# GreenleafLab/NucleoATAC

Measured on AMD Instinct MI355X. Metric: Mbp/s through occ+nuc signal pipeline, higher is better.
Workload: dtype f64

## Files before the change

### nucleoatac_amd/csrc/natac_api.hip

```cpp
#include "../../include/natac.h"
#ifndef NATAC_GNBL
#define NATAC_GNBL 2
#endif
#include "natac_kernels.hpp"
#include "natac_fft_bg.hpp"
#include "natac_occ_fast.hpp"
#include "natac_cand.hpp"
#include "natac_covsweep.hpp"
#include "natac_textz.hpp"
#include "natac_cores.hpp"
#include "natac_writer.hpp"
#include "natac_tabix.hpp"
#include "natac_pack.hpp"
#include "natac_bam.hpp"
#include "natac_bam_dev.hpp"
#include "natac_fragfile.hpp"
#include "natac_fragfile_dev.hpp"
#include "natac_fasta.hpp"
#include "natac_fuzzfit.hpp"
#include "natac_bedtab.hpp"
#include "natac_runtime.hpp"
#include "natac_pwmfit.hpp"
#include "natac_sites.hpp"
#include "natac_cellcounts.hpp"
// ... 6 lines not shown
#include "natac_peaks.hpp"
#include "natac_tracks.hpp"
#include "natac_dropins.hpp"
#include "natac_trackio.hpp"
#include "natac_files.hpp"
#include "natac_store.hpp"
#include "natac_profile.hpp"

#include <algorithm>
#include <cmath>
#include <cstdio>
#include <cstring>
#include <limits>
#include <string>
#include <vector>

using namespace natac;

static int need_nuc_geometry(const natac_batch *b, const char *who) {
    const natac_ctx *c = b->ctx;
    const BatchOutputs &o = b->out;
    if (o.nuc_w < 0 || (o.nuc_w == c->vw && o.nuc_lower == c->vlower && o.nuc_upper == c->vupper)) return NATAC_OK;
    return fail(NATAC_E_STATE, "%s: natac_run_nuc ran with the V-plot geometry lower=%d upper=%d w=%d, the context now holds lower=%d "
                "upper=%d w=%d: run natac_run_nuc again", who, o.nuc_lower, o.nuc_upper, o.nuc_w, c->vlower, c->vupper, c->vw);
}
static int need_occ_geometry(const natac_batch *b, const char *who) {
    const natac_ctx *c = b->ctx;
    const BatchOutputs &o = b->out;
    if (o.occ_step < 0 || (o.occ_step == c->step && o.occ_half == c->halfstep && o.occ_flank == c->flank && o.occ_upper == c->occ_upper))
        return NATAC_OK;
    return fail(NATAC_E_STATE, "%s: natac_run_occ ran with step=%d flank=%d upper=%d, the context now holds step=%d flank=%d upper=%d: "
                "run natac_run_occ again", who, o.occ_step, o.occ_flank, o.occ_upper, c->step, c->flank, c->occ_upper);
}

static int choose_bg_G(const natac_batch *b, int W) {
    const int cand[4] = {7, 9, 13, 17};
    double best = 1e300;
    int bestG = 9;
    const int stride = std::max(1, b->nc / 65536);
    for (int ci = 0; ci < 4; ++ci) {
        const int G = cand[ci], TW = 64 * G;
        double cost = 0;
        for (int i = 0; i < b->nc; i += stride) {
            const int nt = (b->h_len[i] + TW - 1) / TW;
            cost += (double)nt * (TW + (W - 1) * 0.15 * 8);
        }
        if (cost < best) { best = cost; bestG = G; }
    }
    return bestG;
}

static void launch_candidates(natac_ctx *c, const ChunkTable &ct, const VMatDev &vm, const int *d_cc, const int *d_cp, long long n,
                              const double *nuc_cov, const double *norm, const double *bnum, const double *bcov, double *lr,
                              double *var, double *z, const long long *tile_first = nullptr, const int2 *ranges256 = nullptr) {
    const int EW = c->W + ((c->vupper - 2) >> 1) + ((c->vupper - 1) >> 1);
    const int ZN = (((c->vupper - 2) >> 1) + ((c->vupper - 1) >> 1) + 5 + 32) & ~1, ON = (c->W + 1) & ~1;
    const size_t lds4 = ((size_t)4 * CAND_PER_WAVE * ((EW + 1) & ~1) + ZN + ON) * sizeof(double);
    const bool per_wave = c->W <= 2 * WAVE;
    const size_t ldsp = (size_t)4 * CAND_PER_WAVE * CANDP_STRIDE * sizeof(double);
    bool paired = per_wave && bnum && bcov && c->vlower >= 2 && (c->R & 1) == 0 && c->W >= 64 && !vm.has_zero && EW <= CANDP_STRIDE &&
                  !getenv("NATAC_CAND_FULL") && !getenv("NATAC_CAND_OLD");
    if (paired && (c->lrt_gen != c->model_gen || !c->d_lrt)) {
        if (c->d_lrt.size() < (size_t)c->R * c->W && dev_alloc(c->d_lrt, (size_t)c->R * c->W) != NATAC_OK)
            paired = false;
        if (paired) {
            hipLaunchKernelGGL(natac_lr_table, dim3((unsigned)((c->R * c->W + 255) / 256)), dim3(256), 0, c->stream, c->d_vmat, c->d_srow, c->R, c->W,
                               c->d_lrt);
            c->lrt_gen = c->model_gen;
        }
    }
    if (paired && (c->ctab_gen != c->model_gen || !c->d_ctab)) {
        const size_t nd = cand_table_doubles(c->R);
        if (c->d_ctab.size() < nd && dev_alloc(c->d_ctab, nd) != NATAC_OK) paired = false;
        if (paired) {
            hipLaunchKernelGGL(natac_cand_table, dim3((unsigned)((nd / 2 + 255) / 256)), dim3(256), 0, c->stream, c->d_vmat, c->R, c->W, c->d_ctab);
            c->ctab_gen = c->model_gen;
        }
    }
    if (paired) {
        VMatDev vml = vm;
        vml.lrt = c->d_lrt;
        vml.ctab = c->d_ctab;
        const long long per_block = 4 * CAND_PER_WAVE;
        const dim3 grid((unsigned)((n + per_block - 1) / per_block));
        if (c->vlower & 1)
            hipLaunchKernelGGL((natac_candidates_paired<true>), grid, dim3(256), ldsp, c->stream, ct, vml, d_cc, d_cp, (int)n, nuc_cov, norm,
                               bnum, bcov, tile_first, ranges256, lr, var, z);
        else
            hipLaunchKernelGGL((natac_candidates_paired<false>), grid, dim3(256), ldsp, c->stream, ct, vml, d_cc, d_cp, (int)n, nuc_cov, norm,
                               bnum, bcov, tile_first, ranges256, lr, var, z);
        return;
    }
    if (per_wave && lds4 <= 64 * 1024) {
        const long long per_block = 4 * CAND_PER_WAVE;
        if (bnum && bcov && !getenv("NATAC_CAND_FULL"))
            hipLaunchKernelGGL((natac_candidates4<true>), dim3((unsigned)((n + per_block - 1) / per_block)), dim3(256), lds4, c->stream,
                               ct, vm, d_cc, d_cp, (int)n, nuc_cov, norm, bnum, bcov, lr, var, z);
        else
            hipLaunchKernelGGL((natac_candidates4<false>), dim3((unsigned)((n + per_block - 1) / per_block)), dim3(256), lds4, c->stream,
                               ct, vm, d_cc, d_cp, (int)n, nuc_cov, norm, bnum, bcov, lr, var, z);
    } else {
        hipLaunchKernelGGL(natac_candidates, dim3((unsigned)n), dim3(256), (size_t)(EW + 2) * sizeof(double), c->stream, ct, vm, d_cc,
                           d_cp, nuc_cov, norm, lr, var, z);
    }
}

template <int G>
static void launch_bg(natac_batch *b, const ChunkTable &ct, const VMatDev &vm) {
    natac_ctx *c = b->ctx;
    constexpr int W = 121;
    const int PW = 64 * G + W - 1;
    const int EW = PW + ((vm.upper - 2) >> 1) + ((vm.upper - 1) >> 1);
    const size_t lds = ((size_t)((EW + 1) & ~1) + PW) * sizeof(double);
    hipLaunchKernelGGL((natac_background<G, W>), dim3(b->n_tiles_bg), dim3(64), lds, c->stream, ct, b->d_tiles_bg, vm,
                       b->d_track[NATAC_T_NUC_COV], b->d_track[NATAC_T_RAW], b->d_track[NATAC_T_BACKGROUND],
                       b->d_track[NATAC_T_NORM], b->d_bnum, b->d_bcov);
}

struct OccFastLaunch { natac_batch *b; const ChunkTable &ct; const OccFastDev &of; size_t lds_gs, lds_od; int rem; bool rn16; };
template <int STEP, int REM = 0>
static void occ_gsum_launch(const OccFastLaunch &f) {
    if constexpr (REM < STEP) {
        if (f.rem == REM)
            hipLaunchKernelGGL((natac_occ_gsum<STEP, REM>), dim3(f.b->n_tiles_gs), dim3(256), f.lds_gs, f.b->ctx->stream, f.ct, f.b->d_tiles_gs, f.of,
                               f.b->d_blk_off, f.b->total_blocks, f.b->d_gsum);
        else
            occ_gsum_launch<STEP, REM + 1>(f);
    }
}
template <int STEP>
static void occ_fast_launch(const OccFastLaunch &f) {
    natac_batch *b = f.b;
    occ_gsum_launch<STEP>(f);
    auto kd = (f.of.flags & 2) ? (f.rn16 ? natac_occ_decide<STEP, 16, true> : natac_occ_decide<STEP, 4, true>)
                               : (f.rn16 ? natac_occ_decide<STEP, 16, false> : natac_occ_decide<STEP, 4, false>);
    const bool heavy_first = b->ctx->occ_ordered;
    hipLaunchKernelGGL(kd, dim3((b->n_tiles_occ + (heavy_first ? HEAVY_CAP : 0) + 3) / 4), dim3(256), f.lds_od, b->ctx->stream, f.ct, b->d_tiles_occ,
                       b->n_tiles_occ, b->d_ranges_occ, heavy_first ? b->d_order_occ : nullptr, f.of, b->d_blk_off, b->total_blocks, b->d_gsum, b->d_grid[0], b->d_grid[1], b->d_grid[2], b->d_defer,
                       b->d_defer + 1);
}

extern "C" {

// ... 395 lines not shown
    o.zero_flags = c->occ_zero_flags;
    o.b_floor = c->occ_b_floor;
    return o;
}

static int build_tiles(natac_batch *b, int width, PoolBuf<int2> &d_out, int *n_out, bool grid_units = false, int step = 1, int half = 0) {
    std::vector<int2> tiles;
    tiles.reserve((size_t)(b->total_bp / std::max(1, width)) + b->nc);
    for (int i = 0; i < b->nc; ++i) {
        int n = b->h_len[i];
        if (grid_units) n = (b->h_len[i] > half) ? (b->h_len[i] - half + step - 1) / step : 0;
        for (int x = 0; x < n; x += width) tiles.push_back(make_int2(i, x));
    }
    *n_out = (int)tiles.size();
    int rc = dev_upload(b->ctx, d_out, tiles.data(), tiles.size());
    if (rc) return rc;
    HIPCHK(sync_all(b->ctx));
    return NATAC_OK;
}

int natac_batch_create(natac_ctx *c, int32_t nc, const int32_t *chunk_len, const int64_t *frag_off, const int32_t *frag_lpos,
                       const int32_t *frag_ilen, const int64_t *bias_off, const double *bias_log, int32_t bias_left,
                       int32_t bias_right, natac_batch **out) {
    if (!c || !out || !chunk_len || !frag_off) return fail(NATAC_E_ARG, "null argument");
    *out = nullptr;
    if (nc <= 0) return fail(NATAC_E_ARG, "n_chunks must be positive");
    if (bias_log && !bias_off) return fail(NATAC_E_ARG, "bias_log without bias_off");
    if (frag_off[0] != 0) return fail(NATAC_E_ARG, "frag_off[0] must be 0");
    const long long nf = frag_off[nc];
    if (nf > 0 && (!frag_lpos || !frag_ilen)) return fail(NATAC_E_ARG, "fragment arrays are NULL");
    HIPCHK(hipSetDevice(c->device));
    natac_batch *b = new natac_batch();
    b->ctx = c; b->nc = nc; b->nf = nf; b->bias_left = bias_left; b->bias_right = bias_right;
    b->h_len.assign(chunk_len, chunk_len + nc);
    b->h_out_off.resize((size_t)nc + 1);
    b->h_out_off[0] = 0;
    for (int i = 0; i < nc; ++i) {
        if (chunk_len[i] <= 0) { delete b; return fail(NATAC_E_ARG, "chunk %d has length %d", i, chunk_len[i]); }
        if (frag_off[i + 1] < frag_off[i] || frag_off[i + 1] - frag_off[i] > 0x7fffffffLL) {
            delete b; return fail(NATAC_E_ARG, "frag_off not monotone (chunk %d)", i);
        }
        if (bias_off && bias_off[i + 1] - bias_off[i] != (long long)chunk_len[i] + bias_left + bias_right) {
            delete b; return fail(NATAC_E_ARG, "bias slice of chunk %d must cover [start-%d, end+%d)", i, bias_left, bias_right);
        }
        b->h_out_off[i + 1] = b->h_out_off[i] + chunk_len[i];
        b->max_len = std::max(b->max_len, chunk_len[i]);
    }
    b->total_bp = b->h_out_off[nc];
    b->nb = bias_off ? bias_off[nc] : 0;
    auto upload = [&]() -> int {
        int rc;
        if ((rc = dev_upload(c, b->d_len, chunk_len, (size_t)nc)) ||
            (rc = dev_upload(c, b->d_frag_off, (const long long *)frag_off, (size_t)nc + 1)) ||
            (rc = dev_upload(c, b->d_lpos, frag_lpos, (size_t)nf)) || (rc = dev_upload(c, b->d_ilen, frag_ilen, (size_t)nf)) ||
            (rc = dev_alloc(b->d_centre, (size_t)nf)) || (rc = dev_upload(c, b->d_out_off, b->h_out_off.data(), (size_t)nc + 1)))
            return rc;
        if (bias_off) {
            if ((rc = dev_upload(c, b->d_bias_off, (const long long *)bias_off, (size_t)nc + 1))) return rc;
            if (bias_log) rc = dev_upload(c, b->d_bias, bias_log, (size_t)b->nb);
            else rc = dev_alloc(b->d_bias, (size_t)b->nb);
            if (rc) return rc;
        }
        if ((rc = dev_alloc(b->d_status, (size_t)nc))) return rc;
        hipError_t e = hipMemsetAsync(b->d_status, 0, (size_t)nc * sizeof(int), c->stream);
        if (e != hipSuccess) return fail(NATAC_E_HIP, "memset: %s", hipGetErrorString(e));
        if (nf > 0) {
            int blocks = (int)std::min<long long>((nf + 255) / 256, 4096);
            hipLaunchKernelGGL(natac_frag_centres, dim3(blocks), dim3(256), 0, c->stream, b->d_lpos, b->d_ilen, b->d_centre, nf);
        }
        if ((rc = build_tiles(b, 256, b->d_tiles256, &b->n_tiles256))) return rc;
        {
            std::vector<long long> first((size_t)nc + 1, 0);
            for (int i = 0; i < nc; ++i) first[(size_t)i + 1] = first[i] + (chunk_len[i] + 255) / 256;
            if ((rc = dev_upload(c, b->d_tile256_first, first.data(), first.size()))) return rc;
        }
        e = hipStreamSynchronize(c->stream);
        if (e != hipSuccess) return fail(NATAC_E_HIP, "upload: %s", hipGetErrorString(e));
        return NATAC_OK;
    };
    if (int rc = upload()) {
        natac_batch_free(b);
        return rc;
    }
    *out = b;
    return NATAC_OK;
}

int natac_batch_create_from_seq(natac_ctx *c, int32_t nc, const int32_t *chunk_len, const int64_t *frag_off, const int32_t *frag_lpos,
                                const int32_t *frag_ilen, const int64_t *seq_off, const uint8_t *seq, const double *log_pwm,
                                const uint8_t *nucleotides, int nrow, int K, int32_t bias_left, int32_t bias_right, natac_batch **out) {
    if (!c || !out || !chunk_len || !seq_off || !seq || !log_pwm || !nucleotides) return fail(NATAC_E_ARG, "null argument");
    if (nc <= 0 || nrow < 1 || K < 1) return fail(NATAC_E_ARG, "bad argument");
    std::vector<int64_t> boff((size_t)nc + 1, 0);
    for (int i = 0; i < nc; ++i) {
        const int64_t nb = (int64_t)chunk_len[i] + bias_left + bias_right;
        if (seq_off[i + 1] - seq_off[i] != nb + K - 1)
            return fail(NATAC_E_ARG, "sequence window of chunk %d must hold %lld bases ([start-%d-up, end+%d+down))", i, (long long)(nb + K - 1),
                        bias_left, bias_right);
        boff[(size_t)i + 1] = boff[(size_t)i] + nb;
    }
    int rc = natac_batch_create(c, nc, chunk_len, frag_off, frag_lpos, frag_ilen, boff.data(), nullptr, bias_left, bias_right, out);
    if (rc) return rc;
    natac_batch *b = *out;
    DeviceCall dc(c, "pwm score");
    const unsigned char *d_s = dc.upload((const unsigned char *)seq, (size_t)seq_off[nc]);
    const long long *d_so = dc.upload((const long long *)seq_off, (size_t)nc + 1);
    const unsigned char *d_n = dc.upload((const unsigned char *)nucleotides, (size_t)nrow);
    const double *d_p = dc.upload(log_pwm, (size_t)nrow * K);
    if (dc.ok()) {
// ... 577 lines not shown
    for (int r = 1; r < nrow; ++r)
        for (int q = 0; q < r; ++q)
            if (nucleotides[q] == nucleotides[r]) return fail(NATAC_E_ARG, "PWM rows %d and %d have the same letter", q, r);
    if (seq_off[0] != 0) return fail(NATAC_E_ARG, "seq_off[0] must be 0");
    for (int i = 0; i < b->nc; ++i)
        if (seq_off[i + 1] - seq_off[i] != (int64_t)b->h_len[i] + K - 1)
            return fail(NATAC_E_ARG, "sequence window of chunk %d must hold %lld bases (its length + K - 1)", i, (long long)b->h_len[i] + K - 1);
    natac_ctx *c = b->ctx;
    DeviceCall dc(c, "pwm_track");
    int rc;
    if (!dc.ok()) return dc.finish();
    if ((rc = ensure_track(b, NATAC_T_BIAS)) || (rc = ensure_tiles1k(b))) return rc;
    const unsigned char *d_s = dc.upload((const unsigned char *)seq, (size_t)seq_off[b->nc]);
    const long long *d_so = dc.upload((const long long *)seq_off, (size_t)b->nc + 1);
    const unsigned char *d_n = dc.upload((const unsigned char *)nucleotides, (size_t)nrow);
    const double *d_p = dc.upload(log_pwm, (size_t)nrow * K);
    if (dc.ok()) {
        dc.prof_begin(NATAC_K_PWM_TRACK);
        hipLaunchKernelGGL(natac_pwm_track, dim3(b->n_tiles1k), dim3(TR_BLOCK), pwm_track_lds(nrow, K), c->stream, b->d_tiles1k.get(), b->d_len.get(),
                           d_so, d_s, b->d_out_off.get(), d_p, d_n, nrow, K, b->d_track[NATAC_T_BIAS].get());
        dc.prof_end();
        dc.launched();
    }
    if ((rc = dc.finish())) return rc;
    b->out.track[NATAC_T_BIAS] = TS_RUN;
    return NATAC_OK;
}

static int need_candidate_inputs(natac_batch *b) {
    int rc;
    if ((rc = need_track(b, NATAC_T_NUC_COV)) || (rc = need_track(b, NATAC_T_NORM))) return rc;
    if (b->d_bias && !b->d_ebias) return fail(NATAC_E_STATE, "natac_run_nuc must run before the candidate statistics (exp(bias))");
    return NATAC_OK;
}

int natac_run_candidates(natac_batch *b, int64_t n_cand, const int32_t *cand_chunk, const int32_t *cand_pos, double *lr,
                         double *var, double *z) {
    if (!b) return fail(NATAC_E_ARG, "batch is NULL");
    natac_ctx *c = b->ctx;
    int rc = need_candidate_inputs(b);
    if (rc || (rc = need_nuc_geometry(b, "natac_run_candidates"))) return rc;
    if (n_cand < 0 || (n_cand > 0 && (!cand_chunk || !cand_pos || !lr || !var || !z))) return fail(NATAC_E_ARG, "null argument");
    if (n_cand == 0) return NATAC_OK;
    if (n_cand > 0x7fffffffLL) return fail(NATAC_E_ARG, "too many candidates");
    DeviceCall dc(c, "candidates");
    if (!dc.ok()) return dc.finish();
    for (int64_t k = 0; k < n_cand; ++k) {
        const int ci = cand_chunk[k];
        if (ci < 0 || ci >= b->nc || cand_pos[k] < 0 || cand_pos[k] >= b->h_len[ci])
            return fail(NATAC_E_ARG, "candidate %lld out of range (chunk %d pos %d)", (long long)k, ci, cand_pos[k]);
    }
    if ((rc = ensure_srow(c))) return rc;
    const int *d_cc = dc.upload(cand_chunk, (size_t)n_cand), *d_cp = dc.upload(cand_pos, (size_t)n_cand);
    double *d_out = dc.alloc<double>((size_t)3 * n_cand);
    if (dc.ok()) {
        const ChunkTable ct = make_table(b);
        const VMatDev vm = make_vmat(c);
        dc.prof_begin(NATAC_K_CAND);
        launch_candidates(c, ct, vm, d_cc, d_cp, n_cand, b->d_track[NATAC_T_NUC_COV], b->d_track[NATAC_T_NORM],
                          b->out.bg_gen == c->model_gen ? b->d_bnum : nullptr, b->out.bg_gen == c->model_gen ? b->d_bcov : nullptr, d_out,
                          d_out + n_cand,
                          d_out + 2 * n_cand, b->ranges256_w == c->vw ? b->d_tile256_first : nullptr, b->ranges256_w == c->vw ? b->d_ranges256 : nullptr);
        dc.prof_end();
        dc.launched();
    }
    dc.fetch(lr, d_out, (size_t)n_cand);
    dc.fetch(var, d_out + n_cand, (size_t)n_cand);
    dc.fetch(z, d_out + 2 * n_cand, (size_t)n_cand);
    return dc.finish();
}

int natac_run_candidates_cov(natac_batch *b, int64_t n_cand, const int32_t *cand_chunk, const int32_t *cand_pos, int mode,
                             double *var) {
    if (!b) return fail(NATAC_E_ARG, "batch is NULL");
    natac_ctx *c = b->ctx;
    int rc = need_track(b, NATAC_T_NUC_COV);
    if (rc || (rc = need_nuc_geometry(b, "natac_run_candidates_cov"))) return rc;
    if (mode < 0 || mode > 2) return fail(NATAC_E_ARG, "mode must be 0 (closed form), 1 (literal) or 2 (closed form in fp32)");
    if (n_cand < 0 || (n_cand > 0 && (!cand_chunk || !cand_pos || !var))) return fail(NATAC_E_ARG, "null argument");
    if (n_cand == 0) return NATAC_OK;
    DeviceCall dc(c, "candidates_cov");
    if (!dc.ok()) return dc.finish();
    for (int64_t k = 0; k < n_cand; ++k) {
        const int ci = cand_chunk[k];
        if (ci < 0 || ci >= b->nc || cand_pos[k] < 0 || cand_pos[k] >= b->h_len[ci])
            return fail(NATAC_E_ARG, "candidate %lld out of range (chunk %d pos %d)", (long long)k, ci, cand_pos[k]);
    }
    if ((rc = ensure_srow(c))) return rc;
    const int N = c->R * c->W;
    const int NBLK = 64;
    const int64_t SLAB = 2048;
    const ChunkTable ct = make_table(b);
    const VMatDev vm = make_vmat(c);
    const int EW = c->W + ((c->vupper - 2) >> 1) + ((c->vupper - 1) >> 1);
    const int64_t slab = std::min<int64_t>(SLAB, n_cand);
    std::vector<double> part((size_t)slab * NBLK);
    int *d_cc = dc.alloc<int>((size_t)slab), *d_cp = dc.alloc<int>((size_t)slab);
    double *d_p = dc.alloc<double>((size_t)slab * N), *d_out = dc.alloc<double>((size_t)slab * NBLK);
    for (int64_t k0 = 0; k0 < n_cand; k0 += slab) {
        const int64_t m = std::min<int64_t>(slab, n_cand - k0);
        const int per = mode == 1 ? NBLK : 1;
        dc.send(d_cc, cand_chunk + k0, (size_t)m);
        dc.send(d_cp, cand_pos + k0, (size_t)m);
        if (dc.ok()) {
            hipLaunchKernelGGL(natac_cand_window_probs, dim3((unsigned)m), dim3(256), (size_t)(EW + 2) * sizeof(double), c->stream, ct, vm,
                               d_cc, d_cp, d_p);
            dc.launched();
        }
        if (dc.ok()) {
            if (mode == 1)
                hipLaunchKernelGGL(natac_cov_literal_many, dim3(NBLK, (unsigned)m), dim3(256), 0, c->stream, d_p, c->d_vmat, N, d_out);
            else if (mode == 0)
                hipLaunchKernelGGL((natac_cov_closed_many<double>), dim3((unsigned)m), dim3(256), 0, c->stream, d_p, c->d_vmat, N, d_out);
            else
                hipLaunchKernelGGL((natac_cov_closed_many<float>), dim3((unsigned)m), dim3(256), 0, c->stream, d_p, c->d_vmat, N, d_out);
// ... 33 lines not shown
    natac_ctx *c = b->ctx;
    if (order < 1 || order > 255 || sep < 1 || boundary < 0) return fail(NATAC_E_ARG, "bad peak parameters");
    const int maxL = b->max_len;
    if (n_jitter < maxL) return fail(NATAC_E_ARG, "jitter stream (%lld) shorter than the longest chunk (%d)", (long long)n_jitter, maxL);
    HIPCHK(hipSetDevice(c->device));
    HIPCHK(sync_all(c));
    int rc;
    if (with_stats && (rc = ensure_srow(c))) return rc;
    if (!b->d_jitter || b->n_jitter < maxL) {
        if ((rc = dev_upload(c, b->d_jitter, jitter, (size_t)maxL))) return rc;
        HIPCHK(hipStreamSynchronize(c->stream));
        b->n_jitter = maxL;
    } else {
        HIPCHK(hipMemcpyAsync(b->d_jitter, jitter, (size_t)maxL * sizeof(double), hipMemcpyHostToDevice, c->stream));
        HIPCHK(hipStreamSynchronize(c->stream));
    }
    if (b->pk_order != order) {
        std::vector<long long> cap((size_t)b->nc + 1, 0);
        for (int i = 0; i < b->nc; ++i) cap[i + 1] = cap[i] + b->h_len[i] / (order + 1) + 2;
        b->slot_total = cap[b->nc];
        b->d_cap_off.reset(); b->d_slot.reset();
        if ((rc = dev_upload(c, b->d_cap_off, cap.data(), (size_t)b->nc + 1))) return rc;
        HIPCHK(hipStreamSynchronize(c->stream));
        if ((rc = dev_alloc(b->d_slot, (size_t)b->slot_total))) return rc;
        b->pk_order = order;
    }
    if (!b->d_pk_count && (rc = dev_alloc(b->d_pk_count, (size_t)b->nc))) return rc;
    if (!b->d_pk_offs && (rc = dev_alloc(b->d_pk_offs, (size_t)b->nc + 1))) return rc;
    if (form_smooth &&
        (rc = ensure_window(c, c->d_win_nuc, &c->win_nuc_M, &c->win_nuc_sd, b->out.smooth_M, b->out.smooth_sd, &c->win_nuc_sum))) return rc;
    const PeakPlan plan = peaks_plan(maxL, order);
    PeakSearch s{sig_a, sig_b, b->d_jitter, min_signal, boundary, order, sep, b->d_cap_off, b->d_slot, b->d_pk_count, b->d_status,
                 b->d_pk_offs, c->d_win_nuc, c->win_nuc_sum, form_smooth ? b->d_track[NATAC_T_SMOOTH].get() : nullptr};
    if (plan.global_lists) {
        if (b->d_pk_big.size() < (size_t)b->slot_total * 2 + 2 && (rc = dev_alloc(b->d_pk_big, (size_t)b->slot_total * 2 + 2))) return rc;
        s.big_sig = b->d_pk_big;
        s.big_pos = (int *)(b->d_pk_big + b->slot_total);
        s.big_state = (unsigned char *)(s.big_pos + b->slot_total);
    }
    natac_ctx::Ev ev;
    prof_begin(c, NATAC_K_CAND, ev);
    const ChunkTable ct = make_table(b);
    if ((rc = peaks_enqueue(plan, ct, b->nc, s, c->stream))) return rc;
    long long total = 0;
    HIPCHK(hipGetLastError());
    if (form_smooth) b->out.track[NATAC_T_SMOOTH] = TS_RUN;
    HIPCHK(hipMemcpyAsync(&total, b->d_pk_offs + b->nc, sizeof(long long), hipMemcpyDeviceToHost, c->stream));
    HIPCHK(hipStreamSynchronize(c->stream));
    if (total > b->pk_cap) {
        b->d_pk_chunk.reset(); b->d_pk_pos.reset(); b->d_pk_out.reset();
        b->pk_cap = 0;
        const long long cap = total + total / 4 + 16;
        if ((rc = dev_alloc(b->d_pk_chunk, (size_t)cap)) || (rc = dev_alloc(b->d_pk_pos, (size_t)cap)) ||
            (rc = dev_alloc(b->d_pk_out, (size_t)3 * cap))) {
            b->d_pk_chunk.reset(); b->d_pk_pos.reset();
            return rc;
        }
        b->pk_cap = cap;
    }
    if (total > 0) {
        hipLaunchKernelGGL(natac_compact_candidates, dim3((b->nc + 3) / 4), dim3(256), 0, c->stream, b->nc, b->d_pk_count, b->d_pk_offs,
                           b->d_cap_off, b->d_slot, b->d_pk_chunk, b->d_pk_pos);
        if (with_stats) {
            const VMatDev vm = make_vmat(c);
            launch_candidates(c, ct, vm, b->d_pk_chunk, b->d_pk_pos, total, b->d_track[NATAC_T_NUC_COV], b->d_track[NATAC_T_NORM],
                              b->out.bg_gen == c->model_gen ? b->d_bnum : nullptr, b->out.bg_gen == c->model_gen ? b->d_bcov : nullptr,
                              b->d_pk_out, b->d_pk_out + b->pk_cap, b->d_pk_out + 2 * b->pk_cap,
                              b->ranges256_w == c->vw ? b->d_tile256_first : nullptr, b->ranges256_w == c->vw ? b->d_ranges256 : nullptr);
        }
    }
    b->pk_has_stats = with_stats;
    prof_end(c, ev);
    HIPCHK(hipGetLastError());
    b->pk_n = total;
    *n_cand = total;
    return NATAC_OK;
}

int natac_peaks_plan(int32_t max_len, int32_t order, int32_t *kernel, int32_t *bt, int32_t *nj, int32_t *mask, int32_t *global_lists,
                     int32_t *forms_smooth, int32_t *pk_cap, int64_t *lds_bytes) {
    if (!kernel || !bt || !nj || !mask || !global_lists || !forms_smooth || !pk_cap || !lds_bytes) return fail(NATAC_E_ARG, "null argument");
    if (max_len < 1 || order < 1 || order > 255) return fail(NATAC_E_ARG, "natac_peaks_plan: a positive length and an order in 1..255");
    const PeakPlan p = peaks_plan(max_len, order);
    *kernel = p.kernel; *bt = p.bt; *nj = p.nj; *mask = p.mask; *global_lists = p.global_lists; *forms_smooth = p.forms_smooth;
    *pk_cap = p.pk_cap;
    lds_bytes[0] = (int64_t)p.lds; lds_bytes[1] = (int64_t)p.lds_smooth;
    return NATAC_OK;
}

int natac_run_peaks(natac_batch *b, double min_signal, int sep, int boundary, int order, const double *jitter, int64_t n_jitter,
                    int64_t *n_cand) {
    if (!b) return fail(NATAC_E_ARG, "batch is NULL");
    int rc;
    const bool form_smooth = b->out.track[NATAC_T_SMOOTH] == TS_PENDING && peaks_smooth_arm(b, order);
    if ((!form_smooth && (rc = need_track(b, NATAC_T_SMOOTH))) || (rc = need_candidate_inputs(b)) ||
        (rc = need_nuc_geometry(b, "natac_run_peaks"))) return rc;
    return run_peaks_impl(b, b->d_track[NATAC_T_NORM], b->d_track[NATAC_T_SMOOTH], true, min_signal, sep, boundary, order, jitter,
                          n_jitter, n_cand, form_smooth);
}

int natac_run_track_peaks(natac_batch *b, int track, double min_signal, int sep, int boundary, int order, const double *jitter,
                          int64_t n_jitter, int64_t *n_peaks) {
    if (!b) return fail(NATAC_E_ARG, "batch is NULL");
    if (track == NATAC_T_INS) return fail(NATAC_E_ARG, "peak search needs a float64 track");
    int rc = need_track(b, track);
    if (rc) return rc;
    return run_peaks_impl(b, b->d_track[track], nullptr, false, min_signal, sep, boundary, order, jitter, n_jitter, n_peaks);
}

int natac_run_occ_peaks(natac_batch *b, double min_occ, int sep, const double *jitter, int64_t n_jitter, int64_t *n_peaks) {
    if (!b || !n_peaks) return fail(NATAC_E_ARG, "null argument");
    int rc;
    for (int t : {NATAC_T_OCC, NATAC_T_OCC_LOWER, NATAC_T_OCC_UPPER, NATAC_T_OCC_COV}) if ((rc = need_track(b, t))) return rc;
    if ((rc = need_occ_geometry(b, "natac_run_occ_peaks"))) return rc;
    natac_ctx *c = b->ctx;
    const int U = c->occ_upper;
    if (U > 1024) return fail(NATAC_E_ARG, "upper > 1024");
    rc = run_peaks_impl(b, b->d_track[NATAC_T_OCC], nullptr, false, min_occ, sep, sep / 2, 1, jitter, n_jitter, n_peaks);
    if (rc) return rc;
    const long long n = *n_peaks;
// ... 177 lines not shown
```

### nucleoatac_amd/csrc/natac_cand.hpp

```cpp
#pragma once
#include "natac_kernels.hpp"

namespace natac {

__device__ __forceinline__ int row_lower_bound(const int *__restrict__ a, int lo, int hi, int key, int l, int sh) {
    while (__ballot(hi - lo > 16) != 0ull) {
        const int n = hi - lo;
        const bool big = n > 16;
        const int stride = big ? (n + 15) / 16 : 1;
        const int pi = min((l + 1) * stride - 1, max(n - 1, 0));
        const bool less = big && a[lo + pi] < key;
        const int cnt = __popc((unsigned)(__ballot(less) >> sh) & 0xffffu);
        if (big) {
            lo = min(lo + cnt * stride, hi);
            hi = min(lo + stride, hi);
        }
    }
    const int i = lo + l;
    const bool less = (i < hi) && a[i] < key;
    return lo + __popc((unsigned)(__ballot(less) >> sh) & 0xffffu);
}

__global__ void __launch_bounds__(256) natac_lr_table(const double *__restrict__ vmat, const double *__restrict__ srow, int R, int W,
                                                        double *__restrict__ out) {
    const int i = blockIdx.x * 256 + threadIdx.x;
    if (i < R * W) out[i] = log(vmat[i] / srow[i / W]);
}

constexpr int CAND_TAB_PAD = 2;
constexpr int CAND_TAB_PAIR = WAVE * 4;
__host__ __device__ constexpr size_t cand_table_doubles(int R) { return (size_t)((R >> 1) + CAND_TAB_PAD) * CAND_TAB_PAIR; }
__global__ void __launch_bounds__(256) natac_cand_table(const double *__restrict__ vmat, int R, int W, double *__restrict__ out) {
    const int i = blockIdx.x * 256 + threadIdx.x;
    const int k = i >> 7, row = (i >> 6) & 1, l = i & 63;
    if (k >= (R >> 1) + CAND_TAB_PAD) return;
    double v0 = 0.0, v1 = 0.0;
    if (k < (R >> 1)) {
        const double *r = vmat + (size_t)(2 * k + row) * W;
        v0 = r[l];
        if (l + WAVE < W) v1 = r[l + WAVE];
    }
    out[(size_t)i * 2] = v0;
    out[(size_t)i * 2 + 1] = v1;
}

constexpr int CANDP_STRIDE = 376;

template <bool LODD>
__global__ void __launch_bounds__(256) __attribute__((amdgpu_waves_per_eu(3, 3))) natac_candidates_paired(
    ChunkTable ct, VMatDev vm, const int *__restrict__ cand_chunk, const int *__restrict__ cand_pos, int ncand,
    const double *__restrict__ nuc_cov, const double *__restrict__ norm, const double *__restrict__ bnum,
    const double *__restrict__ bcov, const long long *__restrict__ tile_first, const int2 *__restrict__ ranges256,
    double *__restrict__ out_lr, double *__restrict__ out_var, double *__restrict__ out_z) {
    extern __shared__ __attribute__((aligned(16))) double smem[];
    constexpr int Q = CAND_PER_WAVE;
    const int A = (vm.upper - 2) >> 1, Bh = (vm.upper - 1) >> 1;
    const int W = vm.W, R = vm.R;
    const int EW = W + A + Bh;
    constexpr int EWP = CANDP_STRIDE;
    const int wave = threadIdx.x >> 6, lane = threadIdx.x & 63;
    double *Ew = smem + wave * Q * EWP;
    const int k0 = (blockIdx.x * 4 + wave) * Q;
    if (k0 >= ncand) return;
    constexpr int NT = (CANDP_STRIDE + WAVE - 1) / WAVE;
    int chunk[Q], pos[Q];
#pragma unroll
    for (int q = 0; q < Q; ++q) {
        const int k = (k0 + q < ncand) ? k0 + q : k0;
        chunk[q] = cand_chunk[k];
        pos[q] = cand_pos[k];
    }
    double ev[Q][NT];
    if (ct.bias) {
        int nb[Q];
        const double *b[Q];
#pragma unroll
        for (int q = 0; q < Q; ++q) {
            nb[q] = ct.chunk_len[chunk[q]] + ct.bias_left + ct.bias_right;
            b[q] = ct.ebias + ct.bias_off[chunk[q]];
        }
#pragma unroll
        for (int q = 0; q < Q; ++q) {
            const int j0 = pos[q] - vm.w - A + ct.bias_left + lane;
#pragma unroll
            for (int t = 0; t < NT; ++t) ev[q][t] = b[q][min(max(j0 + WAVE * t, 0), nb[q] - 1)];
        }
#pragma unroll
        for (int q = 0; q < Q; ++q) {
            const int j0 = pos[q] - vm.w - A + ct.bias_left + lane;
#pragma unroll
            for (int t = 0; t < NT; ++t) {
                const int j = j0 + WAVE * t;
                ev[q][t] = (j >= 0 && j < nb[q]) ? ev[q][t] : 0.0;
            }
        }
    } else {
#pragma unroll
        for (int q = 0; q < Q; ++q)
#pragma unroll
            for (int t = 0; t < NT; ++t) ev[q][t] = 1.0;
    }
    bool esmall = false;
#pragma unroll
    for (int q = 0; q < Q; ++q) {
        double emin = __builtin_inf();
#pragma unroll
        for (int t = 0; t < NT; ++t) {
            const int u = lane + WAVE * t;
            if (u < EW) {
                Ew[q * EWP + u] = ev[q][t];
                emin = fmin(emin, ev[q][t]);
            }
        }
        esmall |= !(wave_min(emin) > 0x1p-500);
    }
    __builtin_amdgcn_wave_barrier();
    const int c1 = lane, c2 = min(lane + WAVE, W - 1);
    const bool h2 = lane + WAVE < W;
    double a1[Q][2], a2[Q][2];
    double carry[Q][2];
#pragma unroll
    for (int q = 0; q < Q; ++q) { a1[q][0] = a1[q][1] = a2[q][0] = a2[q][1] = 0.0; }
    const int m0 = LODD ? (vm.lower - 1) >> 1 : vm.lower >> 1;
    {
        const int off = LODD ? A + m0 : A - m0 + 1;
#pragma unroll
        for (int q = 0; q < Q; ++q) { carry[q][0] = Ew[q * EWP + c1 + off]; carry[q][1] = Ew[q * EWP + c2 + off]; }
    }
    const double *__restrict__ vmat = vm.mat;
    const int npair = R >> 1;
    constexpr int DSH = LODD ? -1 : 1, DNW = LODD ? 1 : -1;
    constexpr int BSH = DSH < 0 ? 3 : 0, BNW = DNW < 0 ? 3 : 0;
    const int ew0 = wave * Q * EWP;
    int ish1 = ew0 + c1 + (LODD ? A - m0 : A + m0) - BSH, ish2 = ew0 + c2 + (LODD ? A - m0 : A + m0) - BSH;
    int inw1 = ew0 + c1 + (LODD ? A + m0 + 1 : A - m0) - BNW, inw2 = ew0 + c2 + (LODD ? A + m0 + 1 : A - m0) - BNW;
    asm("" : "+v"(ish1), "+v"(ish2), "+v"(inw1), "+v"(inw2));
    struct PairT { double va0, va1, vb0, vb1, sa, sb; };
    constexpr int PAIRB = CAND_TAB_PAIR * (int)sizeof(double);
    const char *ctab = (const char *)vm.ctab;
    unsigned vo = (unsigned)lane * 16u + 4u * PAIRB;
    asm("" : "+v"(vo));
    auto load_pair = [&](int kk, int imm) {
        const double2 *p = (const double2 *)(ctab + (size_t)vo + (ptrdiff_t)imm);
        const double2 a = p[0], b = p[WAVE];
        return PairT{a.x, a.y, b.x, b.y, vm.srow[2 * kk], vm.srow[2 * kk + 1]};
    };
    auto pair_step = [&](const PairT &t, const double (&cin)[Q][2], double (&cout)[Q][2], auto osh, auto onw) {
        const double va0 = t.va0, va1 = t.va1, vb0 = t.vb0, vb1 = t.vb1;
        const double wa0 = t.sa * (va0 * va0), wa1 = t.sa * (va1 * va1);
        const double wb0 = t.sb * (vb0 * vb0), wb1 = t.sb * (vb1 * vb1);
        double s0[Q], s1[Q];
#pragma unroll
        for (int q = 0; q < Q; ++q) {
            s0[q] = smem[ish1 + (q * EWP + osh)]; s1[q] = smem[ish2 + (q * EWP + osh)];
            cout[q][0] = smem[inw1 + (q * EWP + onw)]; cout[q][1] = smem[inw2 + (q * EWP + onw)];
        }
        __builtin_amdgcn_sched_barrier(0);
#pragma unroll
        for (int q = 0; q < Q; ++q) {
            const double n0 = cout[q][0], n1 = cout[q][1];
            a1[q][0] = fma(s0[q], fma(vb0, n0, va0 * cin[q][0]), a1[q][0]);
            a1[q][1] = fma(s1[q], fma(vb1, n1, va1 * cin[q][1]), a1[q][1]);
            a2[q][0] = fma(s0[q], fma(wb0, n0, wa0 * cin[q][0]), a2[q][0]);
            a2[q][1] = fma(s1[q], fma(wb1, n1, wa1 * cin[q][1]), a2[q][1]);
        }
    };
#define NATAC_OFF(J, B, D) std::integral_constant<int, (B) + (J) * (D)>{}
    double carry2[Q][2];
    int k = 0;
    PairT t0 = load_pair(0, -4 * PAIRB), t1 = load_pair(min(1, npair - 1), -3 * PAIRB);
    for (; k + 4 <= npair; k += 4) {
        const PairT u0 = load_pair(min(k + 2, npair - 1), -2 * PAIRB);
        pair_step(t0, carry, carry2, NATAC_OFF(0, BSH, DSH), NATAC_OFF(0, BNW, DNW));
        const PairT u1 = load_pair(min(k + 3, npair - 1), -PAIRB);
        pair_step(t1, carry2, carry, NATAC_OFF(1, BSH, DSH), NATAC_OFF(1, BNW, DNW));
        t0 = load_pair(min(k + 4, npair - 1), 0);
        pair_step(u0, carry, carry2, NATAC_OFF(2, BSH, DSH), NATAC_OFF(2, BNW, DNW));
        t1 = load_pair(min(k + 5, npair - 1), PAIRB);
        pair_step(u1, carry2, carry, NATAC_OFF(3, BSH, DSH), NATAC_OFF(3, BNW, DNW));
        ish1 += 4 * DSH; ish2 += 4 * DSH; inw1 += 4 * DNW; inw2 += 4 * DNW;
        vo += 4u * PAIRB;
    }
    ish1 += BSH; ish2 += BSH; inw1 += BNW; inw2 += BNW;
    for (; k + 2 <= npair; k += 2) {
        pair_step(t0, carry, carry2, NATAC_OFF(0, 0, DSH), NATAC_OFF(0, 0, DNW));
        t0 = load_pair(min(k + 2, npair - 1), -2 * PAIRB);
        pair_step(t1, carry2, carry, NATAC_OFF(1, 0, DSH), NATAC_OFF(1, 0, DNW));
        t1 = load_pair(min(k + 3, npair - 1), -PAIRB);
        ish1 += 2 * DSH; ish2 += 2 * DSH; inw1 += 2 * DNW; inw2 += 2 * DNW;
        vo += 2u * PAIRB;
    }
    if (k < npair) pair_step(t0, carry, carry2, NATAC_OFF(0, 0, DSH), NATAC_OFF(0, 0, DNW));
#undef NATAC_OFF
    bool zero[Q];
#pragma unroll
    for (int q = 0; q < Q; ++q) zero[q] = false;
    if (esmall) {
        for (int r = 0; r < R; ++r) {
            const int i = vm.lower + r;
            const int hl = floor_half(i - 1), hr = floor_half(i);
            const double sr = vm.srow[r];
            const double v1 = vmat[r * W + c1], v2 = vmat[r * W + c2];
#pragma unroll
            for (int q = 0; q < Q; ++q) {
                const double *e = Ew + q * EWP;
                const double b1 = e[c1 + A - hl] * e[c1 + A + hr], b2 = e[c2 + A - hl] * e[c2 + A + hr];
                zero[q] |= (v1 * b1 == 0.0 || sr * b1 == 0.0) || (h2 && (v2 * b2 == 0.0 || sr * b2 == 0.0));
            }
        }
    }
    double tBV2[Q], tB0V[Q];
    bool anyzero[Q];
#pragma unroll
    for (int q = 0; q < Q; ++q) {
        tB0V[q] = wave_sum(a1[q][0] + a1[q][1]);
        tBV2[q] = wave_sum(a2[q][0] + a2[q][1]);
        anyzero[q] = __ballot(zero[q]) != 0ull;
    }
    const int row = lane >> 4, l = lane & 15, sh = 16 * row;
    int mych = chunk[0], myp = pos[0];
    double myB0V = tB0V[0], myBV2 = tBV2[0];
    bool myzero = anyzero[0];
#pragma unroll
    for (int q = 1; q < Q; ++q)
        if (row == q) { mych = chunk[q]; myp = pos[q]; myB0V = tB0V[q]; myBV2 = tBV2[q]; myzero = anyzero[q]; }
    const long long op = ct.out_off[mych] + myp;
    const double tB = bcov[op], tBV = bnum[op];
    const int nfr = (int)(ct.frag_off[mych + 1] - ct.frag_off[mych]);
    const int *cen = ct.centre + ct.frag_off[mych];
    const int *iln = ct.ilen + ct.frag_off[mych];
    int f0, f1;
    if (ranges256) {
        const int2 tr = ranges256[tile_first[mych] + (myp >> 8)];
        const int klo = myp - vm.w, khi = myp + vm.w + 1;
        int below_lo = 0, below_hi = 0;
        int span = tr.y - tr.x;
        span = max(max(__builtin_amdgcn_readlane(span, 0), __builtin_amdgcn_readlane(span, 16)),
                   max(__builtin_amdgcn_readlane(span, 32), __builtin_amdgcn_readlane(span, 48)));
        for (int base = 0; base < span; base += 64) {
            int cv[4];
#pragma unroll
            for (int it = 0; it < 4; ++it) {
                const int i = tr.x + base + 16 * it + l;
                cv[it] = 0x7fffffff;
                if (i < tr.y) cv[it] = cen[i];
            }
#pragma unroll
            for (int it = 0; it < 4; ++it) {
                below_lo += __popc((unsigned)(__ballot(cv[it] < klo) >> sh) & 0xffffu);
                below_hi += __popc((unsigned)(__ballot(cv[it] < khi) >> sh) & 0xffffu);
            }
        }
        f0 = tr.x + below_lo;
        f1 = tr.x + below_hi;
    } else {
        f0 = row_lower_bound(cen, 0, nfr, myp - vm.w, l, sh);
        f1 = row_lower_bound(cen, f0, nfr, myp + vm.w + 1, l, sh);
    }
    const double *__restrict__ lrt = vm.lrt;
    double acc = 0.0, cntf = 0.0;
    int fmax = f1 - f0;
    fmax = max(max(__builtin_amdgcn_readlane(fmax, 0), __builtin_amdgcn_readlane(fmax, 16)),
               max(__builtin_amdgcn_readlane(fmax, 32), __builtin_amdgcn_readlane(fmax, 48)));
    {
        int nn[4], cc[4];
#pragma unroll
        for (int it = 0; it < 4; ++it) {
            const int f = f0 + 16 * it + l;
            nn[it] = -1; cc[it] = 0;
            if (f < f1) { nn[it] = iln[f]; cc[it] = cen[f]; }
        }
        double tv[4];
#pragma unroll
        for (int it = 0; it < 4; ++it) {
            tv[it] = 0.0;
            if (nn[it] >= vm.lower && nn[it] < vm.upper) tv[it] = lrt[(nn[it] - vm.lower) * W + (cc[it] - myp + vm.w)];
        }
#pragma unroll
        for (int it = 0; it < 4; ++it)
            if (nn[it] >= vm.lower && nn[it] < vm.upper) { acc += tv[it]; cntf += 1.0; }
    }
    for (int base = 64; base < fmax; base += 16) {
        const int f = f0 + base + l;
        if (f < f1) {
            const int n = iln[f];
            if (n >= vm.lower && n < vm.upper) { acc += lrt[(n - vm.lower) * W + (cen[f] - myp + vm.w)]; cntf += 1.0; }
        }
    }
    acc = row_sum(acc);
    cntf = row_sum(cntf);
    const double nl = acc, ul = cntf * log(myB0V / tB);
    if (l == 0 && k0 + row < ncand) {
        const double m1 = tBV / tB;
        const double var = cov_reads(nuc_cov[op]) * (myBV2 / tB - m1 * m1);
        out_lr[k0 + row] = myzero ? __builtin_nan("") : (nl - ul);
        out_var[k0 + row] = var;
        out_z[k0 + row] = norm[op] / sqrt(var);
    }
}

}
```

Measured before the change: 3672.

## Split paired candidate kernel into bias-sum pass and per-thread fragment finish kernel

The paired candidate kernel now stops after computing per-candidate bias sums and zero flags, writes them to a scratch buffer, and a new thread-per-candidate finish kernel does the fragment binary search and LR table accumulation using vectorized int4 loads. The bias-window load also drops its per-element bounds clamping, relying on a new host check that the bias flanks are wide enough, and fragment buffers are padded so the vector loads cannot run past the end. This is meant to replace the old wave-row fragment scan with independent per-thread work and to simplify address arithmetic, at the cost of an extra launch and scratch traffic.

```diff
diff --git a/nucleoatac_amd/csrc/natac_api.hip b/nucleoatac_amd/csrc/natac_api.hip
--- a/nucleoatac_amd/csrc/natac_api.hip
+++ b/nucleoatac_amd/csrc/natac_api.hip
@@ -82,14 +82,16 @@
 
 static void launch_candidates(natac_ctx *c, const ChunkTable &ct, const VMatDev &vm, const int *d_cc, const int *d_cp, long long n,
                               const double *nuc_cov, const double *norm, const double *bnum, const double *bcov, double *lr,
-                              double *var, double *z, const long long *tile_first = nullptr, const int2 *ranges256 = nullptr) {
+                              double *var, double *z, double *sums, const long long *tile_first = nullptr,
+                              const int2 *ranges256 = nullptr) {
     const int EW = c->W + ((c->vupper - 2) >> 1) + ((c->vupper - 1) >> 1);
     const int ZN = (((c->vupper - 2) >> 1) + ((c->vupper - 1) >> 1) + 5 + 32) & ~1, ON = (c->W + 1) & ~1;
     const size_t lds4 = ((size_t)4 * CAND_PER_WAVE * ((EW + 1) & ~1) + ZN + ON) * sizeof(double);
     const bool per_wave = c->W <= 2 * WAVE;
     const size_t ldsp = (size_t)4 * CAND_PER_WAVE * CANDP_STRIDE * sizeof(double);
+    const bool flanks = !ct.bias || (ct.bias_left >= c->vw + ((c->vupper - 2) >> 1) && ct.bias_right >= c->vw + ((c->vupper - 1) >> 1));
     bool paired = per_wave && bnum && bcov && c->vlower >= 2 && (c->R & 1) == 0 && c->W >= 64 && !vm.has_zero && EW <= CANDP_STRIDE &&
-                  !getenv("NATAC_CAND_FULL") && !getenv("NATAC_CAND_OLD");
+                  flanks && !getenv("NATAC_CAND_FULL") && !getenv("NATAC_CAND_OLD");
     if (paired && (c->lrt_gen != c->model_gen || !c->d_lrt)) {
         if (c->d_lrt.size() < (size_t)c->R * c->W && dev_alloc(c->d_lrt, (size_t)c->R * c->W) != NATAC_OK)
             paired = false;
@@ -113,12 +115,18 @@
         vml.ctab = c->d_ctab;
         const long long per_block = 4 * CAND_PER_WAVE;
         const dim3 grid((unsigned)((n + per_block - 1) / per_block));
-        if (c->vlower & 1)
-            hipLaunchKernelGGL((natac_candidates_paired<true>), grid, dim3(256), ldsp, c->stream, ct, vml, d_cc, d_cp, (int)n, nuc_cov, norm,
-                               bnum, bcov, tile_first, ranges256, lr, var, z);
-        else
-            hipLaunchKernelGGL((natac_candidates_paired<false>), grid, dim3(256), ldsp, c->stream, ct, vml, d_cc, d_cp, (int)n, nuc_cov, norm,
-                               bnum, bcov, tile_first, ranges256, lr, var, z);
+        const char *e = getenv("NATAC_CAND_RANGES");
+        if (e && e[0] == '0') tile_first = nullptr, ranges256 = nullptr;
+        e = getenv("NATAC_CAND_FINISH");
+        const bool split = !(e && e[0] == '0');
+        const CandSums cs{split ? sums : nullptr, split ? sums + n : nullptr, split ? (unsigned char *)(sums + 2 * n) : nullptr};
+        auto kern = (c->vlower & 1) ? (split ? natac_candidates_paired<true, true> : natac_candidates_paired<true, false>)
+                                    : (split ? natac_candidates_paired<false, true> : natac_candidates_paired<false, false>);
+        hipLaunchKernelGGL(kern, grid, dim3(256), ldsp, c->stream, ct, vml, d_cc, d_cp, (int)n, nuc_cov, norm, bnum, bcov, tile_first,
+                           ranges256, lr, var, z, cs);
+        if (split)
+            hipLaunchKernelGGL(natac_cand_finish, dim3((unsigned)((n + 255) / 256)), dim3(256), 0, c->stream, ct, vml, d_cc, d_cp, (int)n,
+                               nuc_cov, norm, bnum, bcov, tile_first, ranges256, cs, lr, var, z);
         return;
     }
     if (per_wave && lds4 <= 64 * 1024) {
@@ -620,9 +628,10 @@
         int rc;
         if ((rc = dev_upload(c, b->d_len, chunk_len, (size_t)nc)) ||
             (rc = dev_upload(c, b->d_frag_off, (const long long *)frag_off, (size_t)nc + 1)) ||
-            (rc = dev_upload(c, b->d_lpos, frag_lpos, (size_t)nf)) || (rc = dev_upload(c, b->d_ilen, frag_ilen, (size_t)nf)) ||
-            (rc = dev_alloc(b->d_centre, (size_t)nf)) || (rc = dev_upload(c, b->d_out_off, b->h_out_off.data(), (size_t)nc + 1)))
+            (rc = dev_upload(c, b->d_lpos, frag_lpos, (size_t)nf)) || (rc = dev_alloc(b->d_ilen, (size_t)nf + CAND_FRAG_PAD)) ||
+            (rc = dev_alloc(b->d_centre, (size_t)nf + CAND_FRAG_PAD)) || (rc = dev_upload(c, b->d_out_off, b->h_out_off.data(), (size_t)nc + 1)))
             return rc;
+        if (nf) HIPCHK(hipMemcpyAsync(b->d_ilen, frag_ilen, (size_t)nf * sizeof(int), hipMemcpyHostToDevice, c->stream));
         if (bias_off) {
             if ((rc = dev_upload(c, b->d_bias_off, (const long long *)bias_off, (size_t)nc + 1))) return rc;
             if (bias_log) rc = dev_upload(c, b->d_bias, bias_log, (size_t)b->nb);
@@ -1306,15 +1315,14 @@
     }
     if ((rc = ensure_srow(c))) return rc;
     const int *d_cc = dc.upload(cand_chunk, (size_t)n_cand), *d_cp = dc.upload(cand_pos, (size_t)n_cand);
-    double *d_out = dc.alloc<double>((size_t)3 * n_cand);
+    double *d_out = dc.alloc<double>((size_t)3 * n_cand + cand_sums_doubles((size_t)n_cand));
     if (dc.ok()) {
         const ChunkTable ct = make_table(b);
         const VMatDev vm = make_vmat(c);
         dc.prof_begin(NATAC_K_CAND);
         launch_candidates(c, ct, vm, d_cc, d_cp, n_cand, b->d_track[NATAC_T_NUC_COV], b->d_track[NATAC_T_NORM],
                           b->out.bg_gen == c->model_gen ? b->d_bnum : nullptr, b->out.bg_gen == c->model_gen ? b->d_bcov : nullptr, d_out,
-                          d_out + n_cand,
-                          d_out + 2 * n_cand, b->ranges256_w == c->vw ? b->d_tile256_first : nullptr, b->ranges256_w == c->vw ? b->d_ranges256 : nullptr);
+                          d_out + n_cand, d_out + 2 * n_cand, d_out + 3 * n_cand, b->ranges256_w == c->vw ? b->d_tile256_first : nullptr, b->ranges256_w == c->vw ? b->d_ranges256 : nullptr);
         dc.prof_end();
         dc.launched();
     }
@@ -1454,7 +1462,7 @@
         b->pk_cap = 0;
         const long long cap = total + total / 4 + 16;
         if ((rc = dev_alloc(b->d_pk_chunk, (size_t)cap)) || (rc = dev_alloc(b->d_pk_pos, (size_t)cap)) ||
-            (rc = dev_alloc(b->d_pk_out, (size_t)3 * cap))) {
+            (rc = dev_alloc(b->d_pk_out, (size_t)3 * cap + cand_sums_doubles((size_t)cap)))) {
             b->d_pk_chunk.reset(); b->d_pk_pos.reset();
             return rc;
         }
@@ -1467,7 +1475,7 @@
             const VMatDev vm = make_vmat(c);
             launch_candidates(c, ct, vm, b->d_pk_chunk, b->d_pk_pos, total, b->d_track[NATAC_T_NUC_COV], b->d_track[NATAC_T_NORM],
                               b->out.bg_gen == c->model_gen ? b->d_bnum : nullptr, b->out.bg_gen == c->model_gen ? b->d_bcov : nullptr,
-                              b->d_pk_out, b->d_pk_out + b->pk_cap, b->d_pk_out + 2 * b->pk_cap,
+                              b->d_pk_out, b->d_pk_out + b->pk_cap, b->d_pk_out + 2 * b->pk_cap, b->d_pk_out + 3 * b->pk_cap,
                               b->ranges256_w == c->vw ? b->d_tile256_first : nullptr, b->ranges256_w == c->vw ? b->d_ranges256 : nullptr);
         }
     }
diff --git a/nucleoatac_amd/csrc/natac_cand.hpp b/nucleoatac_amd/csrc/natac_cand.hpp
--- a/nucleoatac_amd/csrc/natac_cand.hpp
+++ b/nucleoatac_amd/csrc/natac_cand.hpp
@@ -46,12 +46,18 @@
 
 constexpr int CANDP_STRIDE = 376;
 
-template <bool LODD>
+struct CandSums {
+    double *b0v, *bv2;
+    unsigned char *zero;
+};
+__host__ __device__ constexpr size_t cand_sums_doubles(size_t ncand) { return 2 * ncand + (ncand + 7) / 8; }
+
+template <bool LODD, bool SPLIT>
 __global__ void __launch_bounds__(256) __attribute__((amdgpu_waves_per_eu(3, 3))) natac_candidates_paired(
     ChunkTable ct, VMatDev vm, const int *__restrict__ cand_chunk, const int *__restrict__ cand_pos, int ncand,
     const double *__restrict__ nuc_cov, const double *__restrict__ norm, const double *__restrict__ bnum,
     const double *__restrict__ bcov, const long long *__restrict__ tile_first, const int2 *__restrict__ ranges256,
-    double *__restrict__ out_lr, double *__restrict__ out_var, double *__restrict__ out_z) {
+    double *__restrict__ out_lr, double *__restrict__ out_var, double *__restrict__ out_z, CandSums sums) {
     extern __shared__ __attribute__((aligned(16))) double smem[];
     constexpr int Q = CAND_PER_WAVE;
     const int A = (vm.upper - 2) >> 1, Bh = (vm.upper - 1) >> 1;
@@ -72,27 +78,17 @@
     }
     double ev[Q][NT];
     if (ct.bias) {
-        int nb[Q];
         const double *b[Q];
 #pragma unroll
+        for (int q = 0; q < Q; ++q) b[q] = ct.ebias + ct.bias_off[chunk[q]];
+        int uo[NT];
+#pragma unroll
+        for (int t = 0; t < NT; ++t) uo[t] = min(lane + WAVE * t, EW - 1);
+#pragma unroll
         for (int q = 0; q < Q; ++q) {
-            nb[q] = ct.chunk_len[chunk[q]] + ct.bias_left + ct.bias_right;
-            b[q] = ct.ebias + ct.bias_off[chunk[q]];
-        }
-#pragma unroll
-        for (int q = 0; q < Q; ++q) {
-            const int j0 = pos[q] - vm.w - A + ct.bias_left + lane;
-#pragma unroll
-            for (int t = 0; t < NT; ++t) ev[q][t] = b[q][min(max(j0 + WAVE * t, 0), nb[q] - 1)];
-        }
-#pragma unroll
-        for (int q = 0; q < Q; ++q) {
-            const int j0 = pos[q] - vm.w - A + ct.bias_left + lane;
-#pragma unroll
-            for (int t = 0; t < NT; ++t) {
-                const int j = j0 + WAVE * t;
-                ev[q][t] = (j >= 0 && j < nb[q]) ? ev[q][t] : 0.0;
-            }
+            const double *bq = b[q] + (pos[q] - vm.w - A + ct.bias_left);
+#pragma unroll
+            for (int t = 0; t < NT; ++t) ev[q][t] = bq[uo[t]];
         }
     } else {
 #pragma unroll
@@ -100,10 +96,9 @@
 #pragma unroll
             for (int t = 0; t < NT; ++t) ev[q][t] = 1.0;
     }
-    bool esmall = false;
+    double emin = __builtin_inf();
 #pragma unroll
     for (int q = 0; q < Q; ++q) {
-        double emin = __builtin_inf();
 #pragma unroll
         for (int t = 0; t < NT; ++t) {
             const int u = lane + WAVE * t;
@@ -112,8 +107,8 @@
                 emin = fmin(emin, ev[q][t]);
             }
         }
-        esmall |= !(wave_min(emin) > 0x1p-500);
-    }
+    }
+    const bool esmall = !(wave_min(emin) > 0x1p-500);
     __builtin_amdgcn_wave_barrier();
     const int c1 = lane, c2 = min(lane + WAVE, W - 1);
     const bool h2 = lane + WAVE < W;
@@ -217,6 +212,16 @@
         tBV2[q] = wave_sum(a2[q][0] + a2[q][1]);
         anyzero[q] = __ballot(zero[q]) != 0ull;
     }
+    if constexpr (SPLIT) {
+#pragma unroll
+        for (int q = 0; q < Q; ++q)
+            if (lane == q && k0 + q < ncand) {
+                sums.b0v[k0 + q] = tB0V[q];
+                sums.bv2[k0 + q] = tBV2[q];
+                sums.zero[k0 + q] = anyzero[q] ? 1 : 0;
+            }
+        return;
+    }
     const int row = lane >> 4, l = lane & 15, sh = 16 * row;
     int mych = chunk[0], myp = pos[0];
     double myB0V = tB0V[0], myBV2 = tBV2[0];
@@ -299,4 +304,96 @@
     }
 }
 
-}
+constexpr int CAND_FRAG_PAD = 4;
+struct __attribute__((packed, aligned(4))) Int4U { int v[4]; };
+__device__ __forceinline__ Int4U load_int4(const int *__restrict__ a, int f) { return *(const Int4U *)(a + f); }
+
+__global__ void __launch_bounds__(256) natac_cand_finish(
+    ChunkTable ct, VMatDev vm, const int *__restrict__ cand_chunk, const int *__restrict__ cand_pos, int ncand,
+    const double *__restrict__ nuc_cov, const double *__restrict__ norm, const double *__restrict__ bnum,
+    const double *__restrict__ bcov, const long long *__restrict__ tile_first, const int2 *__restrict__ ranges256, CandSums sums,
+    double *__restrict__ out_lr, double *__restrict__ out_var, double *__restrict__ out_z) {
+    const int k = blockIdx.x * 256 + threadIdx.x;
+    if (k >= ncand) return;
+    const int mych = cand_chunk[k], myp = cand_pos[k];
+    const double myB0V = sums.b0v[k], myBV2 = sums.bv2[k];
+    const bool myzero = sums.zero[k] != 0;
+    const long long op = ct.out_off[mych] + myp;
+    const double tB = bcov[op], tBV = bnum[op];
+    const double cov = nuc_cov[op], nrm = norm[op];
+    const long long fo = ct.frag_off[mych];
+    const int *__restrict__ cen = ct.centre + fo;
+    const int *__restrict__ iln = ct.ilen + fo;
+    int lo = 0, hi = (int)(ct.frag_off[mych + 1] - fo);
+    if (ranges256) {
+        const int2 tr = ranges256[tile_first[mych] + (myp >> 8)];
+        lo = tr.x; hi = tr.y;
+    }
+    const int klo = myp - vm.w, khi = myp + vm.w + 1;
+    int slo = lo, shi = hi;
+    while (shi - slo > 16) {
+        const int stride = (shi - slo + 7) >> 3;
+        int pv[7];
+#pragma unroll
+        for (int j = 1; j < 8; ++j) pv[j - 1] = cen[min(slo + j * stride, shi) - 1];
+        int below = 0;
+#pragma unroll
+        for (int j = 1; j < 8; ++j) below += (slo + j * stride <= shi && pv[j - 1] < klo) ? 1 : 0;
+        slo += below * stride;
+        shi = min(slo + stride, shi);
+    }
+    int f0 = slo;
+    if (slo < shi) {
+        Int4U c[4];
+#pragma unroll
+        for (int g = 0; g < 4; ++g) c[g] = load_int4(cen, min(slo + 4 * g, shi - 1));
+#pragma unroll
+        for (int l = 0; l < 16; ++l) f0 += (slo + l < shi && c[l >> 2].v[l & 3] < klo) ? 1 : 0;
+    }
+    const double *__restrict__ lrt = vm.lrt;
+    const int W = vm.W;
+    double p[16];
+#pragma unroll
+    for (int l = 0; l < 16; ++l) p[l] = 0.0;
+    int cnt = 0;
+    Int4U sz[4], ce[4];
+    auto request = [&](int base) {
+#pragma unroll
+        for (int g = 0; g < 4; ++g) {
+            const int f = min(base + 4 * g, hi - 1);
+            sz[g] = load_int4(iln, f);
+            ce[g] = load_int4(cen, f);
+        }
+    };
+    bool more = f0 < hi;
+    if (more) request(f0);
+    for (int base = f0; more; base += 16) {
+        int idx[16];
+#pragma unroll
+        for (int l = 0; l < 16; ++l) {
+            const int n = sz[l >> 2].v[l & 3], c = ce[l >> 2].v[l & 3];
+            const bool in = base + l < hi && c < khi && n >= vm.lower && n < vm.upper;
+            idx[l] = in ? (n - vm.lower) * W + (c - myp + vm.w) : -1;
+        }
+        more = base + 16 < hi && ce[3].v[3] < khi;
+        double tv[16];
+#pragma unroll
+        for (int l = 0; l < 16; ++l) tv[l] = lrt[max(idx[l], 0)];
+        request(base + 16);
+#pragma unroll
+        for (int l = 0; l < 16; ++l)
+            if (idx[l] >= 0) { p[l] += tv[l]; ++cnt; }
+    }
+    const double q0 = (p[0] + p[1]) + (p[2] + p[3]), q1 = (p[7] + p[6]) + (p[5] + p[4]);
+    const double q3 = (p[15] + p[14]) + (p[13] + p[12]), q2 = (p[8] + p[9]) + (p[10] + p[11]);
+    const double nl = (q0 + q1) + (q3 + q2);
+    const double cntf = (double)cnt;
+    const double ul = cntf * log(myB0V / tB);
+    const double m1 = tBV / tB;
+    const double var = cov_reads(cov) * (myBV2 / tB - m1 * m1);
+    out_lr[k] = myzero ? __builtin_nan("") : (nl - ul);
+    out_var[k] = var;
+    out_z[k] = nrm / sqrt(var);
+}
+
+}
```

Measured after the change: 3697 (median of 6 runs). About the same (+0.7%).
